# pyg-team/pytorch_geometric

Measured on AMD Instinct MI355X. Metric: edges/sec (fwd+bwd) 3-layer SAGE, ogbn-products shape, higher is better.
Workload: dtype f32

## Files before the change

include/pyg_amd.h:

```cpp
#ifndef PYG_AMD_H
#define PYG_AMD_H

#include <stddef.h>
#include <stdint.h>

#ifdef __cplusplus
extern "C" {
#endif

#define PYGAMD_API __attribute__((visibility("default")))

#define PYGAMD_ABI_VERSION 11

typedef enum {
  PYGAMD_OK = 0,
  PYGAMD_ERR_INVALID_ARG = 1,
  PYGAMD_ERR_UNSUPPORTED = 2,
  PYGAMD_ERR_WORKSPACE = 3,
  PYGAMD_ERR_HIP = 4
} pygamd_status;

typedef enum { PYGAMD_IDX_I32 = 0, PYGAMD_IDX_I64 = 1 } pygamd_idx_dtype;

typedef enum { PYGAMD_X_DENSE = 0, PYGAMD_X_COMPRESSED = 1 } pygamd_x_format;
// ... 429 lines not shown
                                                    const int64_t* frontier_time,
                                                    const int64_t* item_begin,
                                                    const int64_t* et_table, int n_et,
                                                    uint64_t timed_mask, int replace,
                                                    int strategy, void* lo_out, void* hi_out,
                                                    void* cnt_out, void* stream);
PYGAMD_API int pygamd_hetero_sample_neighbors_temporal(const void* row, const void* perm,
                                                       int idx_dtype, const void* frontier,
                                                       const void* lo, const void* hi,
                                                       const void* offsets,
                                                       const int64_t* item_begin,
                                                       const int64_t* et_table, int n_et,
                                                       uint64_t seed, int flags, void* src_out,
                                                       void* col_out, void* edge_out,
                                                       void* fpos_out, void* stream);

PYGAMD_API int pygamd_hetero_spmm(const void* rowptr, const void* col, int idx_dtype,
                                  const int64_t* row_begin, const float* const* x,
                                  float* const* out, const int64_t* et_table, int n_et, int64_t F,
                                  int32_t* err_flag, void* stream);
PYGAMD_API int pygamd_hetero_spmm_backward(const void* rowptr_t, const void* col_t,
                                           const void* rowptr, int idx_dtype,
                                           const int64_t* row_begin, const float* const* grad,
                                           const int64_t* et_table, int n_et,
                                           const int64_t* src_begin, float* const* grad_x,
                                           const int64_t* ld_grad_x, int n_nt, int64_t F,
                                           void* stream);

PYGAMD_API int pygamd_hgt_supported(int64_t H, int64_t D);
PYGAMD_API int pygamd_hgt_workspace_bytes(const int64_t* et_table, int n_et, int64_t H, int64_t D,
                                          size_t* bytes );
PYGAMD_API int pygamd_hgt_relation_forward(const float* const* k, const float* const* v,
                                           const int64_t* et_table, int n_et, const float* wk,
                                           const float* wv, int64_t T, int64_t H, int64_t D,
                                           float* kv, void* stream);
PYGAMD_API int pygamd_hgt_relation_backward(const float* const* k, const float* const* v,
                                            const int64_t* et_table, int n_et, const float* wk,
                                            const float* wv, int64_t T, int64_t H, int64_t D,
                                            const float* grad_kv, float* const* grad_k,
                                            float* const* grad_v, const int64_t* nt_table,
                                            int n_nt, float* grad_wk, float* grad_wv,
                                            void* workspace, size_t workspace_bytes,
                                            void* stream);

PYGAMD_API int pygamd_multi_reduce_csr(const void* rowptr, const void* perm, int idx_dtype,
                                       const float* x, int64_t ldx, int64_t n_rows, int64_t F,
                                       float* out_sum, float* out_sq, float* out_min,
                                       float* out_max, int64_t ldo, void* stream);

#define PYGAMD_GEMM_FP32 0
#define PYGAMD_GEMM_SPLIT_BF16 1
PYGAMD_API int pygamd_set_gemm_mode(int mode);
PYGAMD_API int pygamd_get_gemm_mode(void);
PYGAMD_API int pygamd_linear_nt_workspace_bytes(int64_t M, int64_t N_out, int64_t K_red,
                                                size_t* bytes );
PYGAMD_API int pygamd_linear_forward(const float* x, int64_t ldx, const float* w, int64_t ldw,
                                     const float* bias, int64_t M, int64_t K, int64_t N, int relu,
                                     int accumulate, float* out, int64_t ldo, void* workspace,
                                     size_t workspace_bytes, void* stream);
PYGAMD_API int pygamd_linear_dgrad(const float* g, int64_t ldg, const float* w_t, int64_t ldwt,
                                   const float* row_scale, int64_t n_scaled, int64_t M, int64_t N,
                                   int64_t K, int accumulate, const float* relu_mask,
                                   int64_t ld_mask, const uint32_t* relu_bits, int64_t ld_bits,
                                   float* out, int64_t ldo, void* stream);
PYGAMD_API int pygamd_linear_dgrad2(const float* g, int64_t ldg, const float* w_t, int64_t ldwt,
                                    const float* row_scale, int64_t n_scaled, int64_t M,
                                    int64_t N, int64_t K, int accumulate, const float* relu_mask,
                                    int64_t ld_mask, const uint32_t* relu_bits, int64_t ld_bits,
                                    float* out, int64_t ldo, float* out_scaled, int64_t ld_scaled,
                                    void* workspace, size_t workspace_bytes, void* stream);
PYGAMD_API int pygamd_linear_wgrad_workspace_bytes(int64_t M, int64_t N, int64_t K,
                                                   size_t* bytes );
PYGAMD_API int pygamd_linear_wgrad(const float* g, int64_t ldg, const float* x, int64_t ldx,
                                   int64_t M, int64_t N, int64_t K, int accumulate,
                                   int wgs_per_cu ,
                                   float* out, int64_t ldo, float* bias_grad, void* workspace,
                                   size_t workspace_bytes, void* stream);
PYGAMD_API int pygamd_linear_wgrad2(const float* g, int64_t ldg, const float* x, int64_t ldx,
                                    int64_t K1, const float* x2, int64_t ldx2, int64_t K2,
                                    int64_t M, int64_t N, int accumulate, int wgs_per_cu,
                                    float* out, int64_t ldo, float* bias_grad, void* workspace,
                                    size_t workspace_bytes, void* stream);

PYGAMD_API int pygamd_slots_max_fanout(void);
PYGAMD_API int pygamd_slots_max_hops(void);
PYGAMD_API int pygamd_slots_seed(const void* seeds, int idx_dtype, int64_t B,
                                 const int64_t* epoch_dev, int64_t* local_map, int64_t* node_g,
                                 void* stream);
PYGAMD_API int pygamd_slots_sample(const void* colptr, const void* row, int idx_dtype,
                                   const int64_t* node_g, int64_t frontier_base,
                                   int64_t n_frontier, int fanout, int64_t slot_base, int64_t B,
                                   uint64_t seed, int hop, const int64_t* epoch_dev,
                                   int64_t* local_map, int64_t* src_g, int32_t* row_end,
                                   float* inv_cnt, void* stream);
PYGAMD_API int pygamd_slots_resolve(const int64_t* src_g, int64_t slot_base, int64_t n_slots,
                                    int64_t B, const int64_t* epoch_dev,
                                    const int64_t* local_map, int32_t* src_id,
                                    int64_t* node_g, int32_t* const* counts ,
                                    int n_counts, void* stream);
PYGAMD_API int pygamd_slots_gather(const float* x, int64_t ldx, int64_t F, const int64_t* node_g,
                                   int64_t n_rows, float* out, int64_t ldo, void* stream);
PYGAMD_API int pygamd_slots_transpose(const int64_t* src_g, const int32_t* src_id, int hops,
                                      const int32_t* fanout ,
                                      const int64_t* bases , int n_csr,
                                      const int64_t* n_slots ,
                                      const int64_t* n_src_rows ,
// ... 65 lines not shown
```

pytorch_geometric_amd/_build.py:

```python
import os
import shutil
import subprocess
import sys
from concurrent.futures import ThreadPoolExecutor

PKG_DIR = os.path.dirname(os.path.abspath(__file__))
CSRC_DIR = os.path.join(PKG_DIR, 'csrc')
LIB_DIR = os.path.join(PKG_DIR, 'lib')
LIB_PATH = os.path.join(LIB_DIR, 'libpyg_amd.so')
LAB_LIB_PATH = os.path.join(LIB_DIR, 'libpyg_amd_lab.so')
BUILD_DIR = os.path.join(os.path.dirname(PKG_DIR), 'build', 'pyg_amd')
SOURCES = ['capi.hip', 'graph.hip', 'spmm.hip', 'scatter.hip', 'softmax.hip', 'segmm.hip',
           'sample.hip', 'minibatch.hip', 'train.hip', 'gemm.hip', 'sage_fused.hip',
           'hetero_conv.hip', 'gatv2.hip', 'transformer.hip', 'hgt.hip', 'gine.hip']
LAB_SOURCES = SOURCES + ['sage_fused_lab.hip']
LAB_FLAGS = {'gemm.hip': ['-DPYGAMD_LAB=1']}
ARCH = 'gfx950'
FLAGS = [f'--offload-arch={ARCH}', '-O3', '-std=c++17', '-fPIC', '-fvisibility=hidden',
         '-Wall', '-Wno-unused-function']
FLAGS += os.environ.get('PYGAMD_EXTRA_HIPCC_FLAGS', '').split()
EXTRA_FLAGS = {}


def find_hipcc():
    cand = shutil.which('hipcc') or '/opt/rocm/bin/hipcc'
    return cand if os.path.exists(cand) else None


STAMP_PATH = LIB_PATH + '.stamp'
LAB_STAMP_PATH = LAB_LIB_PATH + '.stamp'


BINDING_SRC = os.path.join(CSRC_DIR, 'torch_binding.cpp')
BINDING_PATH = os.path.join(LIB_DIR, 'libpyg_amd_torch.so')
BINDING_STAMP = BINDING_PATH + '.stamp'


def source_hash():
    import hashlib
    h = hashlib.sha1()
    paths = sorted(os.path.join(CSRC_DIR, f) for f in os.listdir(CSRC_DIR)
                   if f != os.path.basename(BINDING_SRC))
    paths.append(os.path.join(os.path.dirname(PKG_DIR), 'include', 'pyg_amd.h'))
    paths.append(os.path.join(os.path.dirname(PKG_DIR), 'include', 'pyg_amd_lab.h'))
    for p in paths:
        if os.path.isfile(p):
            h.update(os.path.basename(p).encode())
            with open(p, 'rb') as f:
                h.update(f.read())
    h.update(' '.join(FLAGS).encode())
    h.update(repr(sorted(EXTRA_FLAGS.items())).encode())
    return h.hexdigest()


def is_stale():
    if not (os.path.exists(LIB_PATH) and os.path.exists(STAMP_PATH)):
        return True
    with open(STAMP_PATH) as f:
        return f.read().strip() != source_hash()


def lab_is_stale():
    if not (os.path.exists(LAB_LIB_PATH) and os.path.exists(LAB_STAMP_PATH)):
        return True
    with open(LAB_STAMP_PATH) as f:
        return f.read().strip() != source_hash()
# ... 110 lines not shown
```

pytorch_geometric_amd/_lib.py:

```python
import ctypes
import os
from ctypes import (POINTER, Structure, c_char_p, c_double, c_float, c_int, c_int32, c_int64,
                    c_size_t, c_uint64, c_void_p)

from . import _build

ABI_VERSION = 11
X_DENSE, X_COMPRESSED = 0, 1
AGG_GIVEN = 2
IDX_I32, IDX_I64 = 0, 1
SUM, MEAN, MIN, MAX, MUL, ANY = 0, 1, 2, 3, 4, 5
REDUCE_IDS = {'sum': SUM, 'add': SUM, 'mean': MEAN, 'min': MIN, 'amin': MIN, 'max': MAX,
              'amax': MAX, 'mul': MUL, 'any': ANY}


class PygAmdError(RuntimeError):
    pass


class SpmmArgs(Structure):
    _fields_ = [
        ('rowptr', c_void_p), ('col', c_void_p), ('eid', c_void_p), ('w', c_void_p),
        ('src_scale', c_void_p), ('x', c_void_p), ('out', c_void_p), ('arg_out', c_void_p),
        ('n_rows', c_int64), ('n_src', c_int64), ('F', c_int64), ('ldx', c_int64),
# ... 41 lines not shown
    'pygamd_ptr2index': (c_int, [_P, c_int, c_int64, c_int64, _P, _P]),
    'pygamd_index_minmax': (c_int, [_P, c_int, c_int64, _P, _P]),
    'pygamd_permute_index': (c_int, [_P, c_int, _P, c_int64, _P, _P]),
    'pygamd_cast_index': (c_int, [_P, c_int64, c_int, _P, _P]),
    'pygamd_index_guard': (c_int, [_P, c_int, c_int64, c_int64, _P, c_int, _P, _P]),
    'pygamd_cumsum_workspace_bytes': (c_int, [c_int, c_int64, POINTER(c_size_t)]),
    'pygamd_cumsum': (c_int, [_P, c_int, c_int64, _P, _P, c_size_t, _P]),
    'pygamd_hub_plan_workspace_bytes': (c_int, [c_int, c_int64, POINTER(c_size_t)]),
    'pygamd_hub_plan': (c_int, [_P, c_int, c_int64, c_int64, c_int64, _P, _P, c_int64,
                                POINTER(c_int64), POINTER(c_int64), _P, c_size_t, _P]),
    'pygamd_rows_compress': (c_int, [_P, c_int64, c_int64, c_int64, _P, c_int64, _P]),
    'pygamd_rows_pack': (c_int, [_P, c_int64, c_int64, c_int64, _P, _P, c_int64, c_int64, _P,
                                 c_int64, c_int64, _P, _P, _P]),
    'pygamd_spmm_csr_workspace_bytes': (c_int, [POINTER(SpmmArgs), POINTER(c_size_t)]),
    'pygamd_spmm_csr': (c_int, [POINTER(SpmmArgs), _P, c_size_t, _P]),
    'pygamd_spmm_csr_tie_count': (c_int, [_P, _P, c_int, _P, c_int64, _P, c_int64, c_int64,
                                          c_int64, c_int, _P, _P]),
    'pygamd_spmm_csr_minmax_backward': (c_int, [_P, _P, c_int, _P, c_int64, _P, _P, _P, c_int64,
                                                c_int64, c_int64, _P, c_int64, _P]),
    'pygamd_spmm_csr_minmax_backward_dst': (c_int, [_P, _P, c_int, _P, c_int64, _P, c_int64, _P,
                                                    c_int64, c_int64, c_int64, c_int64, c_int, _P,
                                                    c_int64, _P]),
    'pygamd_multi_reduce_csr': (c_int, [_P, _P, c_int, _P, c_int64, c_int64, c_int64, _P, _P, _P,
                                        _P, c_int64, _P]),
    'pygamd_minmax_backward_src_workspace_bytes': (c_size_t, [c_int64, c_int64, c_int64]),
    'pygamd_spmm_csr_minmax_backward_src': (c_int, [_P, _P, _P, _P, _P, c_int, _P, _P, c_int64, _P,
                                                    c_int64, _P, c_int64, c_int64, c_int64,
                                                    c_int64, c_int64, c_int, _P, c_size_t, _P,
                                                    c_int64, _P]),
    'pygamd_spmm_csr_minmax_backward_arg': (c_int, [_P, _P, c_int, _P, _P, c_int64, _P, c_int64, _P,
                                                    c_int64, c_int64, c_int64, c_int64, c_int, _P,
                                                    c_int64, _P]),
    'pygamd_sddmm_csr': (c_int, [_P, _P, _P, c_int, _P, c_int64, _P, c_int64, c_int64, c_int64,
                                 c_int32, c_int32, _P, _P]),
    'pygamd_sddmm_spmm_csr': (c_int, [_P, _P, _P, c_int, _P, c_int64, _P, c_int64, c_int64,
                                      c_int64, c_int32, c_int32, _P, _P, _P, c_int64, _P]),
    'pygamd_colsum': (c_int, [_P, c_int64, c_int64, c_int64, _P, _P]),
    'pygamd_bias_act': (c_int, [_P, c_int64, _P, c_int64, c_int64, c_int, _P, c_int64, _P]),
    'pygamd_relu_backward_colsum': (c_int, [_P, c_int64, _P, c_int64, c_int64, c_int64, _P,
                                            c_int64, _P, _P]),
    'pygamd_sage_layer_forward_supported': (c_int, [c_int64, c_int64, c_int]),
    'pygamd_sage_layer_forward': (c_int, [POINTER(SpmmArgs), _P, c_int64, _P, c_int64, _P, c_int64,
                                          c_int, c_int, _P, c_int64, _P, c_int64, _P, c_size_t,
                                          _P]),
    'pygamd_sage_layer_fused': (c_int, [POINTER(SpmmArgs), POINTER(SageFusedArgs), _P, c_size_t,
                                        _P]),
    'pygamd_sage_layer_fused_workspace_bytes': (c_int, [POINTER(SpmmArgs), POINTER(SageFusedArgs),
                                                        POINTER(c_size_t)]),
    'pygamd_linear_nt_workspace_bytes': (c_int, [c_int64, c_int64, c_int64, POINTER(c_size_t)]),
    'pygamd_linear_forward': (c_int, [_P, c_int64, _P, c_int64, _P, c_int64, c_int64, c_int64,
                                      c_int, c_int, _P, c_int64, _P, c_size_t, _P]),
    'pygamd_set_gemm_mode': (c_int, [c_int]),
    'pygamd_get_gemm_mode': (c_int, []),
    'pygamd_linear_dgrad': (c_int, [_P, c_int64, _P, c_int64, _P, c_int64, c_int64, c_int64,
                                    c_int64, c_int, _P, c_int64, _P, c_int64, _P, c_int64, _P]),
    'pygamd_linear_dgrad2': (c_int, [_P, c_int64, _P, c_int64, _P, c_int64, c_int64, c_int64,
                                     c_int64, c_int, _P, c_int64, _P, c_int64, _P, c_int64, _P,
                                     c_int64, _P, c_size_t, _P]),
    'pygamd_linear_wgrad_workspace_bytes': (c_int, [c_int64, c_int64, c_int64,
                                                    POINTER(c_size_t)]),
    'pygamd_linear_wgrad': (c_int, [_P, c_int64, _P, c_int64, c_int64, c_int64, c_int64, c_int,
                                    c_int, _P, c_int64, _P, _P, c_size_t, _P]),
    'pygamd_linear_wgrad2': (c_int, [_P, c_int64, _P, c_int64, c_int64, _P, c_int64, c_int64,
                                     c_int64, c_int64, c_int, c_int, _P, c_int64, _P, _P,
                                     c_size_t, _P]),
    'pygamd_segment_matmul_tile_rows': (c_int, []),
    'pygamd_segment_matmul_workspace_bytes': (c_int, [c_int64, c_int64, c_int64,
                                                      POINTER(c_size_t)]),
    'pygamd_segment_matmul': (c_int, [_P, c_int64, _P, _P, c_int64, c_int64, c_int64, c_int64,
                                      _P, c_int64, c_int64, c_int64, c_int64, _P, c_int64, _P,
                                      c_size_t, _P]),
    'pygamd_segment_matmul_wgrad': (c_int, [_P, c_int64, _P, c_int64, _P, _P, c_int64, c_int64,
                                            c_int64, c_int64, c_int64, _P, _P]),
    'pygamd_sample_max_fanout': (c_int, []),
    'pygamd_sample_neighbors': (c_int, [_P, _P, c_int, _P, c_int64, _P, c_int64, c_uint64, c_int,
                                        _P, _P, _P, _P, _P]),
    'pygamd_sample_neighbors_weighted': (c_int, [_P, _P, c_int, _P, _P, c_int64, _P, c_int64,
                                                 c_uint64, c_int, _P, _P, _P, _P, _P]),
    'pygamd_sample_temporal_window': (c_int, [_P, _P, c_int, _P, c_int, _P, _P, c_int64, c_int64,
                                              c_int, c_int, _P, _P, _P, _P, _P]),
    'pygamd_sample_neighbors_temporal': (c_int, [_P, c_int, _P, c_int64, _P, _P, _P, c_int64,
                                                 c_uint64, c_int, _P, _P, _P, _P, _P]),
    'pygamd_slots_max_fanout': (c_int, []),
    'pygamd_slots_max_hops': (c_int, []),
    'pygamd_slots_seed': (c_int, [_P, c_int, c_int64, _P, _P, _P, _P]),
    'pygamd_slots_sample': (c_int, [_P, _P, c_int, _P, c_int64, c_int64, c_int, c_int64, c_int64,
                                    c_uint64, c_int, _P, _P, _P, _P, _P, _P]),
    'pygamd_slots_resolve': (c_int, [_P, c_int64, c_int64, c_int64, _P, _P, _P, _P, _P, c_int,
                                     _P]),
    'pygamd_slots_gather': (c_int, [_P, c_int64, c_int64, _P, c_int64, _P, c_int64, _P]),
    'pygamd_slots_transpose': (c_int, [_P, _P, c_int, _P, _P, c_int, _P, _P, _P, _P, _P, _P, _P]),
    'pygamd_cross_entropy_step_workspace_bytes': (c_int, [c_int64, _P]),
    'pygamd_cross_entropy_step': (c_int, [_P, c_int64, _P, c_int64, c_int64, c_int64, _P, _P, _P,
                                          c_int64, _P, _P, c_size_t, _P, _P, _P]),
    'pygamd_adam_step': (c_int, [_P, _P, _P, _P, c_int64, _P, c_int64, c_double, c_double,
                                 c_double, c_double, c_double, c_double, _P, c_int, _P, _P, _P,
                                 _P, _P]),
    'pygamd_edge_key': (c_int, [_P, _P, c_int, c_int64, c_int64, c_int, _P, _P]),
    'pygamd_run_flags': (c_int, [_P, c_int64, _P, _P]),
    'pygamd_edge_unkey': (c_int, [_P, _P, _P, c_int64, c_int64, c_int, c_int, _P, _P, _P, _P]),
    'pygamd_sample_counts': (c_int, [_P, c_int, _P, c_int64, c_int64, c_int, _P, _P, _P]),
    'pygamd_relabel': (c_int, [c_int, _P, c_int, c_int64, _P, _P, _P, c_int64, _P, _P, _P]),
    'pygamd_sample_negatives': (c_int, [c_int64, c_int64, c_uint64, _P, _P, _P, _P, c_int64,
                                        c_int64, c_int, _P, _P]),
    'pygamd_unique_inverse': (c_int, [_P, _P, c_int, c_int64, _P, _P, c_size_t, _P, _P, _P, _P]),
    'pygamd_hetero_sample_counts': (c_int, [_P, c_int, _P, _P, _P, c_int, c_int, _P, _P]),
# ... 53 lines not shown
                                                 c_int64, c_float, _P, _P, _P]),
    'pygamd_gatv2_supported': (c_int, [c_int64, c_int64]),
    'pygamd_gatv2_workspace_bytes': (c_int, [c_int64, c_int64, c_int64, POINTER(c_size_t)]),
    'pygamd_gatv2_forward': (c_int, [_G, _P, _P, _P, c_int64, c_int64, c_int64, c_float, _P, _P, _P,
                                     c_size_t, _P]),
    'pygamd_gatv2_backward_dst': (c_int, [_G, _P, _P, _P, _P, _P, _P, _P, c_int64, c_int64, c_int64,
                                          c_float, _P, _P, _P, _P, c_size_t, _P]),
    'pygamd_gatv2_backward_src': (c_int, [_G, _P, _P, _P, _P, _P, _P, _P, c_int64, c_int64, c_int64,
                                          c_float, _P, _P, c_size_t, _P]),
    'pygamd_transformer_supported': (c_int, [c_int64, c_int64]),
    'pygamd_transformer_workspace_bytes': (c_int, [c_int64, c_int64, c_int64,
                                                   POINTER(c_size_t)]),
    'pygamd_transformer_forward': (c_int, [_G, _P, _P, _P, c_int64, c_int64, c_int64, c_int64,
                                           c_float, _P, _P, _P, c_size_t, _P]),
    'pygamd_transformer_backward_dst': (c_int, [_G, _P, _P, c_int64, _P, _P, _P, _P, c_int64,
                                                c_int64, c_int64, c_float, _P, _P, _P, c_size_t,
                                                _P]),
    'pygamd_transformer_backward_src': (c_int, [_G, _P, _P, _P, _P, _P, c_int64, c_int64, c_int64,
                                                c_float, _P, _P, c_int64, _P, c_size_t, _P]),
    'pygamd_transformer_edge_supported': (c_int, [c_int64, c_int64, c_int64]),
    'pygamd_transformer_edge_workspace_bytes': (c_int, [c_int64, c_int64, c_int64, c_int64,
                                                        POINTER(c_size_t)]),
    'pygamd_transformer_edge_forward': (c_int, [_G, _P, _P, _P, c_int64, _P, _P, c_int64, c_int64,
                                                c_int64, c_int64, c_float, _P, _P, _P, _P, c_size_t,
                                                _P]),
    'pygamd_transformer_edge_backward_dst': (c_int, [_G, _P, _P, c_int64, _P, _P, _P, _P, _P, _P,
                                                     _P, _P, c_int64, c_int64, c_int64, c_int64,
                                                     c_float, _P, _P, _P, _P, _P, c_size_t, _P]),
    'pygamd_gine_supported': (c_int, [c_int64, c_int64]),
    'pygamd_gine_workspace_bytes': (c_int, [c_int64, c_int64, c_int64, POINTER(c_size_t)]),
    'pygamd_gine_forward': (c_int, [_G, _P, _P, c_int64, _P, c_int64, _P, _P, _P, _P, c_int64,
                                    c_int64, c_int64, _P, _P, c_size_t, _P]),
    'pygamd_gine_backward': (c_int, [_G, _P, _P, c_int64, _P, _P, _P, _P, c_int64, c_int64, c_int64,
                                     _P, _P, _P, _P, _P, c_size_t, _P]),
}

LAB_SIGNATURES = {
    'pygamd_lab_sage_layer_fused': (c_int, [POINTER(SpmmArgs), POINTER(SageFusedArgs), c_int,
                                            c_int, _P, c_size_t, _P]),
    'pygamd_lab_set_wgrad_variant': (c_int, [c_int]),
    'pygamd_lab_copy': (c_int, [_P, _P, c_int64, c_int, c_int, _P]),
}

_lib = None
_lab = None
_use_lab = False


def lib_path():
    return _build.LIB_PATH


GEMM_MODES = {'fp32': 0, 'split': 1}


def _open(path, signatures):
    lib = ctypes.CDLL(path)
    for name, (restype, argtypes) in signatures:
        fn = getattr(lib, name)
        fn.restype = restype
        fn.argtypes = argtypes
    if lib.pygamd_abi_version() != ABI_VERSION:
        raise PygAmdError(f'ABI mismatch: {path} reports {lib.pygamd_abi_version()}')
    return lib


def _default_mode():
    mode = os.environ.get('PYGAMD_GEMM_MODE', 'split')
    if mode not in GEMM_MODES:
        raise PygAmdError(f"PYGAMD_GEMM_MODE must be one of {sorted(GEMM_MODES)}, got '{mode}'")
    return GEMM_MODES[mode]


def load():
    global _lib
    if _use_lab:
        return load_lab()
    if _lib is not None:
        return _lib
    path = _build.LIB_PATH
    if _build.is_stale():
        if _build.find_hipcc() is not None and os.environ.get('PYG_AMD_NO_BUILD') != '1':
            _build.build_library(verbose=False)
        elif not os.path.exists(path):
            raise PygAmdError(
                f"{path} is missing and hipcc is unavailable: run "
                f"`python -c 'import __graft_entry__ as g; g.build()'` on a machine with ROCm. "
                f"There is no CPU fallback for the pytorch_geometric_amd kernels.")
    lib = _open(path, list(SIGNATURES.items()))
    lib.pygamd_set_gemm_mode(_default_mode())
    _lib = lib
    return lib


def load_lab():
    global _lab
    if _lab is not None:
        return _lab
    path = _build.LAB_LIB_PATH
    if _build.lab_is_stale():
        if _build.find_hipcc() is not None and os.environ.get('PYG_AMD_NO_BUILD') != '1':
            _build.build_lab_library(verbose=False)
        elif not os.path.exists(path):
            raise PygAmdError(f"{path} is missing and hipcc is unavailable (the laboratory "
                              f"build: `python -m pytorch_geometric_amd._build`)")
    lab = _open(path, list(SIGNATURES.items()) + list(LAB_SIGNATURES.items()))
    lab.pygamd_set_gemm_mode(_lib.pygamd_get_gemm_mode() if _lib is not None else _default_mode())
    _lab = lab
    return lab


def use_lab(flag: bool) -> None:
    global _use_lab
    _use_lab = bool(flag)
    if _use_lab:
        load_lab()


def lab_active() -> bool:
    return _use_lab


def loaded():
    if _lib is None and _lab is None:
        load()
    return [l for l in (_lib, _lab) if l is not None]


def check(rc, what=''):
    if rc != 0:
        lib = load()
        msg = lib.pygamd_status_string(rc).decode()
        extra = f' (hipError {lib.pygamd_last_hip_error()})' if rc == 4 else ''
        raise PygAmdError(f'{what or "pygamd call"} failed: {msg}{extra}')
```

pytorch_geometric_amd/_native.py:

```python
import collections
import ctypes
import os
import threading
from typing import Optional, Tuple

import torch
from torch import Tensor

from . import _compiled, _lib
from ._lib import REDUCE_IDS, Csr, PygAmdError, SpmmArgs, check

HUB_THRESHOLD = 1024
HUB_CHUNK = int(os.environ.get('PYGAMD_HUB_CHUNK', '256'))


def _require_device(*tensors):
    for t in tensors:
        if t is not None and not t.is_cuda:
            raise PygAmdError(
                'pytorch_geometric_amd kernels need HIP device tensors (got a '
                f'{t.device} tensor); there is no CPU fallback on this path')


def _idx_dtype(t: Tensor) -> int:
# ... 1623 lines not shown
                                     'compressed_out': compressed_out is not None}}, ev0, ev1))
    return out


def cross_entropy_rows(logits: Tensor, target: Tensor, index: Optional[Tensor] = None):
    _require_device(logits, target, index)
    x = _f32_rows(logits, 'logits')
    N, C = x.shape
    if target.dtype != torch.int64 or target.dim() != 1 or target.numel() != N \
            or not target.is_contiguous():
        raise ValueError(f"'target' must hold one contiguous int64 label per row of 'logits' "
                         f"({N}), got {target.dtype} {tuple(target.shape)}")
    if index is not None and (index.dtype != torch.int64 or index.dim() != 1
                              or not index.is_contiguous()):
        raise ValueError("'index' must be a contiguous 1-D int64 tensor")
    B = N if index is None else index.numel()
    if B == 0 or C == 0:
        raise ValueError('cross_entropy_rows needs at least one row and one class')
    lib = _lib.load()
    grad = torch.empty(B, C, dtype=torch.float32, device=x.device)
    loss = torch.empty((), dtype=torch.float32, device=x.device)
    nbytes = ctypes.c_size_t(0)
    check(lib.pygamd_cross_entropy_step_workspace_bytes(B, ctypes.byref(nbytes)))
    ws = torch.empty(nbytes.value, dtype=torch.uint8, device=x.device)
    ring, slot, err = _index_flag(x.device, True)
    check(lib.pygamd_cross_entropy_step(_p(x), _ld(x), _p(index), N, B, C, _p(target), _p(index),
                                        _p(grad), C, _p(loss), _p(ws), nbytes.value, _p(err),
                                        None, _stream(x)), 'cross_entropy_rows')
    _index_flag_done(ring, slot, err, "cross_entropy: a target outside [0, C) (or an 'index' "
                     "entry outside the rows of the logits)", C, target)
    return loss, grad


def set_gemm_mode(mode: str) -> str:
    lib = _lib.load()
    if mode not in _lib.GEMM_MODES:
        raise ValueError(f"mode must be one of {sorted(_lib.GEMM_MODES)}, got '{mode}'")
    prev = get_gemm_mode()
    for each in _lib.loaded():
        check(each.pygamd_set_gemm_mode(_lib.GEMM_MODES[mode]), 'set_gemm_mode')
    return prev


def lab_set_wgrad_variant(variant: int) -> None:
    check(_lib.load_lab().pygamd_lab_set_wgrad_variant(int(variant)), 'lab_set_wgrad_variant')
    _lib.use_lab(int(variant) != 0)


def get_gemm_mode() -> str:
    code = _lib.load().pygamd_get_gemm_mode()
    return next(k for k, v in _lib.GEMM_MODES.items() if v == code)


def linear_dgrad(g: Tensor, w_t: Tensor, row_scale: Optional[Tensor] = None, n_scaled: int = 0,
                 out: Optional[Tensor] = None, accumulate: bool = False,
                 relu_mask: Optional[Tensor] = None, relu_bits: Optional[Tensor] = None,
                 out_scaled: Optional[Tensor] = None) -> Tensor:
    _require_device(g, w_t, row_scale, out, relu_mask, relu_bits, out_scaled)
    if relu_mask is not None and relu_bits is not None:
        raise ValueError("pass at most one of 'relu_mask' / 'relu_bits'")
    C = _compiled.ops()
    if C is not None and _plain(g, w_t, relu_mask, out, out_scaled) \
            and g.size(1) == w_t.size(1):
        M, K = g.size(0), w_t.size(0)
        ok = ((out is None or (out.shape == (M, K) and (K <= 1 or out.stride(1) == 1)))
              and (relu_mask is None or tuple(relu_mask.shape) == (M, K))
              and (out_scaled is None or (row_scale is not None and not accumulate
                                          and out_scaled.shape == (M, K)
                                          and (K <= 1 or out_scaled.stride(1) == 1))))
        if ok:
            _check_bits(relu_bits, M, K)
            if out is None:
                out = torch.empty(M, K, dtype=torch.float32, device=g.device)
            with _timed({'kind': 'gemm', 'op': 'dgrad', 'M': M, 'N': K, 'K': g.size(1)}, g):
                C.linear_dgrad(g, w_t, row_scale, n_scaled, out, accumulate, relu_mask,
                               relu_bits, out_scaled)
            return out
    lib = _lib.load()
    g2, w2 = _f32_rows(g, 'grad'), _f32_rows(w_t, 'weight_t')
    M, N = g2.shape
    K = w2.size(0)
    if w2.size(1) != N:
        raise ValueError(f"'grad' has {N} columns but 'weight_t' expects {w2.size(1)}")
    if out is None:
        out = torch.empty(M, K, dtype=torch.float32, device=g.device)
    if row_scale is not None:
        row_scale = row_scale.contiguous()
    if out_scaled is not None:
        if row_scale is None or accumulate:
            raise ValueError("'out_scaled' needs 'row_scale' and no 'accumulate'")
        if out_scaled.shape != (M, K) or out_scaled.dtype != torch.float32 \
                or (K > 1 and out_scaled.stride(1) != 1):
            raise ValueError("'out_scaled' must be a float32 [M, K] tensor with unit inner stride")
    m2 = None
    _check_bits(relu_bits, M, K)
    if relu_mask is not None:
        m2 = _f32_rows(relu_mask, 'relu_mask')
        if tuple(m2.shape) != (M, K):
            raise ValueError(f"'relu_mask' must be [{M}, {K}], got {tuple(m2.shape)}")
    ws, ws_bytes = _nt_workspace(lib, M, K, N, g.device)
    with _timed({'kind': 'gemm', 'op': 'dgrad', 'M': M, 'N': K, 'K': N}, g):
        check(lib.pygamd_linear_dgrad2(_p(g2), _ld(g2), _p(w2), _ld(w2), _p(row_scale),
                                       n_scaled if row_scale is not None else 0, M, N, K,
                                       int(accumulate), _p(m2), _ld(m2) if m2 is not None else 0,
                                       _p(relu_bits),
                                       relu_bits.size(1) if relu_bits is not None else 0,
# ... 795 lines not shown
```

pytorch_geometric_amd/csrc/gemm.hip:

```cpp
#include "split_bf16.h"
#include "../../include/pyg_amd_lab.h"

namespace pygamd {

typedef float f32x16 __attribute__((ext_vector_type(16)));
typedef float f32x4 __attribute__((ext_vector_type(4)));

struct SplitFrag {
  bf16x8 p[3];
};

__device__ __forceinline__ SplitFrag split_frag(const f32x4& v0, const f32x4& v1) {
  u32x4 w[3];
#pragma unroll
  for (int q = 0; q < 4; ++q) {
    const float x0 = q < 2 ? v0[2 * q] : v1[2 * q - 4];
    const float x1 = q < 2 ? v0[2 * q + 1] : v1[2 * q - 3];
    uint32_t t[3];
    split_pair(x0, x1, t);
    w[0][q] = t[0];
    w[1][q] = t[1];
    w[2][q] = t[2];
  }
  SplitFrag f;
#pragma unroll
  for (int t = 0; t < 3; ++t) f.p[t] = __builtin_bit_cast(bf16x8, w[t]);
  return f;
}

__device__ __forceinline__ void split_term(int t, const SplitFrag& a, const SplitFrag& b,
                                           f32x16& acc) {
  acc = __builtin_amdgcn_mfma_f32_32x32x16_bf16(a.p[kSplitTa[t]], b.p[kSplitTb[t]], acc, 0, 0, 0);
}

constexpr int kGK = 32;
constexpr int kGLD = kGK + 4;

struct GemmNT {
  const float* __restrict__ a;
  const float* __restrict__ b;
  const float* __restrict__ bias;
  const float* __restrict__ row_scale;
  const float* __restrict__ mask;
  const uint32_t* __restrict__ mask_bits;
  int64_t ldmb;
  float* __restrict__ c;
  float* __restrict__ c2;
  int64_t ldc2;
  int64_t M, lda, ldb, ldc, ldm;
  int N, K;
  int relu;
  int n_scaled;
  int accumulate;
  int tiles_m, tiles_n;
  int split;
  int ksplits, k_per_split;
  float* __restrict__ partial;
};

__device__ __forceinline__ void nt_tile_of_block(const GemmNT& p, int& tm, int& tn) {
  const int64_t b = blockIdx.x;
  const int64_t per_xcd = gridDim.x >> 3;
  const int64_t q = (b & 7) * per_xcd + (b >> 3);
  tm = static_cast<int>(q / p.tiles_n);
  tn = static_cast<int>(q - static_cast<int64_t>(tm) * p.tiles_n);
}

template <int WM, int WN, int TM, int TN, bool VEC, bool SPLIT>
__global__ void __launch_bounds__(kBlock, 2) gemm_nt_kernel(GemmNT p) {
  static_assert(WM * WN == 4, "four waves per workgroup");
  constexpr int BM = WM * TM * 32, BN = WN * TN * 32;
  constexpr int A_LD4 = BM * (kGK / 4) / kBlock;
  constexpr int B_LD4 = (BN * (kGK / 4) + kBlock - 1) / kBlock;
  extern __shared__ __align__(16) float smem[];
  float* As = smem;
  float* Bs = smem + 2 * BM * kGLD;
  int tile_m, tile_n;
  nt_tile_of_block(p, tile_m, tile_n);
  if (tile_m >= p.tiles_m) return;
  const int64_t m0 = static_cast<int64_t>(tile_m) * BM;
  const int n0 = tile_n * BN;
  const int wave = threadIdx.x >> 6, lane = threadIdx.x & 63;
  const int wm = wave / WN, wn = wave % WN;
  const int li = lane & 31, lh = lane >> 5;
  const int kb = p.ksplits > 1 ? static_cast<int>(blockIdx.y) * p.k_per_split : 0;
  const int ke = p.ksplits > 1 ? (kb + p.k_per_split < p.K ? kb + p.k_per_split : p.K) : p.K;

  const int kq = threadIdx.x & 7;
  const int r0 = threadIdx.x >> 3;
  const float* pa[A_LD4];
  const float* pb[B_LD4];
  bool okb[B_LD4];
#pragma unroll
  for (int q = 0; q < A_LD4; ++q) {
    int64_t row = m0 + r0 + 32 * q;
    row = row < p.M ? row : p.M - 1;
    pa[q] = p.a + row * p.lda;
  }
#pragma unroll
  for (int q = 0; q < B_LD4; ++q) {
    int row = n0 + r0 + 32 * q;
    okb[q] = row < p.N && (BN % 32 == 0 || r0 + 32 * q < BN);
    row = row < p.N ? row : p.N - 1;
    pb[q] = p.b + static_cast<int64_t>(row) * p.ldb;
  }
  f32x4 ra[A_LD4], rb[B_LD4];
  auto load_chunk = [&](int k0) {
    const int k = k0 + 4 * kq;
    if (VEC) {
      const int kc = k < ke ? k : 0;
#pragma unroll
// ... 1076 lines not shown
  return PYGAMD_OK;
}

static int g_gemm_mode = 0;
#ifdef PYGAMD_LAB
static int g_wgrad_variant = 0;
#else
constexpr int g_wgrad_variant = 0;
#endif

constexpr int kFillTiles = 128;
struct NtShape {
  int tile;
  int ksplits;
  int k_per_split;
};
static NtShape nt_shape(int64_t M, int N, int K, bool allow_splitk) {
  NtShape s;
  s.tile = N > 96 ? 0 : N > 64 ? 1 : N > 32 ? 2 : 3;
  s.ksplits = 1;
  s.k_per_split = K;
  const int bn[5] = {128, 96, 64, 32, 64};
  int64_t tiles = ceil_div(M, 128) * ceil_div(N, bn[s.tile]);
  if (tiles >= kFillTiles) return s;
  if (N > 32) {
    s.tile = 4;
    tiles = ceil_div(M, 64) * ceil_div(N, 64);
  }
  if (allow_splitk && tiles < kFillTiles && K >= 128) {
    int want = static_cast<int>(ceil_div(2 * kFillTiles, tiles));
    const int most = K / 64;
    want = want < most ? want : most;
    want = want < 32 ? want : 32;
    if (want > 1) {
      s.k_per_split = static_cast<int>(round_up(ceil_div(K, want), kGK));
      s.ksplits = static_cast<int>(ceil_div(K, s.k_per_split));
    }
  }
  return s;
}

static int run_nt(GemmNT p, void* workspace, size_t workspace_bytes, hipStream_t st) {
  if (p.M == 0 || p.N == 0) return PYGAMD_OK;
  p.split = g_gemm_mode == PYGAMD_GEMM_SPLIT_BF16 ? 1 : 0;
  const bool vec = (p.K % 4 == 0) && (p.lda % 4 == 0) && (p.ldb % 4 == 0) && aligned16p(p.a) &&
                   aligned16p(p.b);
  NtShape sh = nt_shape(p.M, p.N, p.K, workspace != nullptr);
  if (sh.ksplits > 1 &&
      workspace_bytes < static_cast<size_t>(sh.ksplits) * p.M * p.N * sizeof(float))
    sh = nt_shape(p.M, p.N, p.K, false);
  p.ksplits = sh.ksplits;
  p.k_per_split = sh.k_per_split;
  p.partial = sh.ksplits > 1 ? static_cast<float*>(workspace) : nullptr;
  switch (sh.tile) {
    case 0: return launch_nt<2, 2, 2, 2>(p, vec, st);
    case 1: return launch_nt<4, 1, 1, 3>(p, vec, st);
    case 2: return launch_nt<4, 1, 1, 2>(p, vec, st);
    case 3: return launch_nt<4, 1, 1, 1>(p, vec, st);
    default: return launch_nt<2, 2, 1, 1>(p, vec, st);
  }
}

}

using namespace pygamd;

extern "C" {

int pygamd_set_gemm_mode(int mode) {
  if (mode != PYGAMD_GEMM_FP32 && mode != PYGAMD_GEMM_SPLIT_BF16) return PYGAMD_ERR_INVALID_ARG;
  g_gemm_mode = mode;
  return PYGAMD_OK;
}

int pygamd_get_gemm_mode(void) { return g_gemm_mode; }

#ifdef PYGAMD_LAB
int pygamd_lab_set_wgrad_variant(int variant) {
  if (variant < 0 || variant > 127 || ((variant & 1) && variant != 1))
    return PYGAMD_ERR_INVALID_ARG;
  g_wgrad_variant = variant;
  return PYGAMD_OK;
}
#endif

int pygamd_linear_forward(const float* x, int64_t ldx, const float* w, int64_t ldw,
                          const float* bias, int64_t M, int64_t K, int64_t N, int relu,
                          int accumulate, float* out, int64_t ldo, void* workspace,
                          size_t workspace_bytes, void* stream) {
  if (M < 0 || K < 0 || N < 0 || K > INT32_MAX || N > INT32_MAX || ldx < K || ldw < K ||
      ldo < N)
    return PYGAMD_ERR_INVALID_ARG;
  if (M == 0 || N == 0) return PYGAMD_OK;
  if (!out || (K > 0 && (!x || !w))) return PYGAMD_ERR_INVALID_ARG;
  GemmNT p = {};
  p.a = x; p.b = w; p.bias = bias; p.row_scale = nullptr; p.mask = nullptr; p.c = out;
  p.M = M; p.lda = ldx; p.ldb = ldw; p.ldc = ldo; p.ldm = 0;
  p.N = static_cast<int>(N); p.K = static_cast<int>(K);
  p.relu = relu ? 1 : 0; p.n_scaled = 0; p.accumulate = accumulate ? 1 : 0;
  return run_nt(p, workspace, workspace_bytes, as_stream(stream));
}

int pygamd_linear_dgrad2(const float* g, int64_t ldg, const float* w_t, int64_t ldwt,
                         const float* row_scale, int64_t n_scaled, int64_t M, int64_t N,
                         int64_t K, int accumulate, const float* relu_mask, int64_t ld_mask,
                         const uint32_t* relu_bits, int64_t ld_bits, float* out, int64_t ldo,
// ... 186 lines not shown
```

Baseline: 4.503 billion.

## Add persistent streaming NT GEMM kernel with LDS-resident split-bf16 weights

```diff
diff --git a/include/pyg_amd.h b/include/pyg_amd.h
--- a/include/pyg_amd.h
+++ b/include/pyg_amd.h
@@ -505,6 +505,12 @@
 #define PYGAMD_GEMM_SPLIT_BF16 1
 PYGAMD_API int pygamd_set_gemm_mode(int mode);
 PYGAMD_API int pygamd_get_gemm_mode(void);
+#define PYGAMD_STREAM_OFF 0
+#define PYGAMD_STREAM_AUTO 1
+#define PYGAMD_STREAM_FORCE 2
+PYGAMD_API int pygamd_set_stream_mode(int mode);
+PYGAMD_API int pygamd_get_stream_mode(void);
+PYGAMD_API int64_t pygamd_stream_launch_count(void);
 PYGAMD_API int pygamd_linear_nt_workspace_bytes(int64_t M, int64_t N_out, int64_t K_red,
                                                 size_t* bytes );
 PYGAMD_API int pygamd_linear_forward(const float* x, int64_t ldx, const float* w, int64_t ldw,
diff --git a/pytorch_geometric_amd/_build.py b/pytorch_geometric_amd/_build.py
--- a/pytorch_geometric_amd/_build.py
+++ b/pytorch_geometric_amd/_build.py
@@ -11,7 +11,7 @@
 LAB_LIB_PATH = os.path.join(LIB_DIR, 'libpyg_amd_lab.so')
 BUILD_DIR = os.path.join(os.path.dirname(PKG_DIR), 'build', 'pyg_amd')
 SOURCES = ['capi.hip', 'graph.hip', 'spmm.hip', 'scatter.hip', 'softmax.hip', 'segmm.hip',
-           'sample.hip', 'minibatch.hip', 'train.hip', 'gemm.hip', 'sage_fused.hip',
+           'sample.hip', 'minibatch.hip', 'train.hip', 'gemm.hip', 'stream_nt.hip', 'sage_fused.hip',
            'hetero_conv.hip', 'gatv2.hip', 'transformer.hip', 'hgt.hip', 'gine.hip']
 LAB_SOURCES = SOURCES + ['sage_fused_lab.hip']
 LAB_FLAGS = {'gemm.hip': ['-DPYGAMD_LAB=1']}
diff --git a/pytorch_geometric_amd/_lib.py b/pytorch_geometric_amd/_lib.py
--- a/pytorch_geometric_amd/_lib.py
+++ b/pytorch_geometric_amd/_lib.py
@@ -117,6 +117,9 @@
                                       c_int, c_int, _P, c_int64, _P, c_size_t, _P]),
     'pygamd_set_gemm_mode': (c_int, [c_int]),
     'pygamd_get_gemm_mode': (c_int, []),
+    'pygamd_set_stream_mode': (c_int, [c_int]),
+    'pygamd_get_stream_mode': (c_int, []),
+    'pygamd_stream_launch_count': (c_int64, []),
     'pygamd_linear_dgrad': (c_int, [_P, c_int64, _P, c_int64, _P, c_int64, c_int64, c_int64,
                                     c_int64, c_int, _P, c_int64, _P, c_int64, _P, c_int64, _P]),
     'pygamd_linear_dgrad2': (c_int, [_P, c_int64, _P, c_int64, _P, c_int64, c_int64, c_int64,
@@ -276,6 +279,7 @@
 
 
 GEMM_MODES = {'fp32': 0, 'split': 1}
+STREAM_MODES = {'off': 0, 'auto': 1, 'force': 2}
 
 
 def _open(path, signatures):
@@ -294,6 +298,14 @@
     if mode not in GEMM_MODES:
         raise PygAmdError(f"PYGAMD_GEMM_MODE must be one of {sorted(GEMM_MODES)}, got '{mode}'")
     return GEMM_MODES[mode]
+
+
+def _default_stream_mode():
+    mode = os.environ.get('PYGAMD_STREAM_MODE', 'auto')
+    if mode not in STREAM_MODES:
+        raise PygAmdError(f"PYGAMD_STREAM_MODE must be one of {sorted(STREAM_MODES)}, got "
+                          f"'{mode}'")
+    return STREAM_MODES[mode]
 
 
 def load():
@@ -313,6 +325,7 @@
                 f"There is no CPU fallback for the pytorch_geometric_amd kernels.")
     lib = _open(path, list(SIGNATURES.items()))
     lib.pygamd_set_gemm_mode(_default_mode())
+    lib.pygamd_set_stream_mode(_default_stream_mode())
     _lib = lib
     return lib
 
@@ -330,6 +343,8 @@
                               f"build: `python -m pytorch_geometric_amd._build`)")
     lab = _open(path, list(SIGNATURES.items()) + list(LAB_SIGNATURES.items()))
     lab.pygamd_set_gemm_mode(_lib.pygamd_get_gemm_mode() if _lib is not None else _default_mode())
+    lab.pygamd_set_stream_mode(_lib.pygamd_get_stream_mode() if _lib is not None
+                               else _default_stream_mode())
     _lab = lab
     return lab
 
diff --git a/pytorch_geometric_amd/_native.py b/pytorch_geometric_amd/_native.py
--- a/pytorch_geometric_amd/_native.py
+++ b/pytorch_geometric_amd/_native.py
@@ -1699,6 +1699,25 @@
     return next(k for k, v in _lib.GEMM_MODES.items() if v == code)
 
 
+def set_stream_mode(mode: str) -> str:
+    _lib.load()
+    if mode not in _lib.STREAM_MODES:
+        raise ValueError(f"mode must be one of {sorted(_lib.STREAM_MODES)}, got '{mode}'")
+    prev = get_stream_mode()
+    for each in _lib.loaded():
+        check(each.pygamd_set_stream_mode(_lib.STREAM_MODES[mode]), 'set_stream_mode')
+    return prev
+
+
+def get_stream_mode() -> str:
+    code = _lib.load().pygamd_get_stream_mode()
+    return next(k for k, v in _lib.STREAM_MODES.items() if v == code)
+
+
+def stream_launch_count() -> int:
+    return int(_lib.load().pygamd_stream_launch_count())
+
+
 def linear_dgrad(g: Tensor, w_t: Tensor, row_scale: Optional[Tensor] = None, n_scaled: int = 0,
                  out: Optional[Tensor] = None, accumulate: bool = False,
                  relu_mask: Optional[Tensor] = None, relu_bits: Optional[Tensor] = None,
diff --git a/pytorch_geometric_amd/csrc/gemm.hip b/pytorch_geometric_amd/csrc/gemm.hip
--- a/pytorch_geometric_amd/csrc/gemm.hip
+++ b/pytorch_geometric_amd/csrc/gemm.hip
@@ -1,62 +1,10 @@
-#include "split_bf16.h"
+#include "gemm_nt.h"
 #include "../../include/pyg_amd_lab.h"
 
 namespace pygamd {
-
-typedef float f32x16 __attribute__((ext_vector_type(16)));
-typedef float f32x4 __attribute__((ext_vector_type(4)));
-
-struct SplitFrag {
-  bf16x8 p[3];
-};
-
-__device__ __forceinline__ SplitFrag split_frag(const f32x4& v0, const f32x4& v1) {
-  u32x4 w[3];
-#pragma unroll
-  for (int q = 0; q < 4; ++q) {
-    const float x0 = q < 2 ? v0[2 * q] : v1[2 * q - 4];
-    const float x1 = q < 2 ? v0[2 * q + 1] : v1[2 * q - 3];
-    uint32_t t[3];
-    split_pair(x0, x1, t);
-    w[0][q] = t[0];
-    w[1][q] = t[1];
-    w[2][q] = t[2];
-  }
-  SplitFrag f;
-#pragma unroll
-  for (int t = 0; t < 3; ++t) f.p[t] = __builtin_bit_cast(bf16x8, w[t]);
-  return f;
-}
-
-__device__ __forceinline__ void split_term(int t, const SplitFrag& a, const SplitFrag& b,
-                                           f32x16& acc) {
-  acc = __builtin_amdgcn_mfma_f32_32x32x16_bf16(a.p[kSplitTa[t]], b.p[kSplitTb[t]], acc, 0, 0, 0);
-}
 
 constexpr int kGK = 32;
 constexpr int kGLD = kGK + 4;
-
-struct GemmNT {
-  const float* __restrict__ a;
-  const float* __restrict__ b;
-  const float* __restrict__ bias;
-  const float* __restrict__ row_scale;
-  const float* __restrict__ mask;
-  const uint32_t* __restrict__ mask_bits;
-  int64_t ldmb;
-  float* __restrict__ c;
-  float* __restrict__ c2;
-  int64_t ldc2;
-  int64_t M, lda, ldb, ldc, ldm;
-  int N, K;
-  int relu;
-  int n_scaled;
-  int accumulate;
-  int tiles_m, tiles_n;
-  int split;
-  int ksplits, k_per_split;
-  float* __restrict__ partial;
-};
 
 __device__ __forceinline__ void nt_tile_of_block(const GemmNT& p, int& tm, int& tn) {
   const int64_t b = blockIdx.x;
@@ -1239,6 +1187,7 @@
   p.ksplits = sh.ksplits;
   p.k_per_split = sh.k_per_split;
   p.partial = sh.ksplits > 1 ? static_cast<float*>(workspace) : nullptr;
+  if (stream_nt_takes(p, vec)) return stream_nt_launch(p, st);
   switch (sh.tile) {
     case 0: return launch_nt<2, 2, 2, 2>(p, vec, st);
     case 1: return launch_nt<4, 1, 1, 3>(p, vec, st);
diff --git a/pytorch_geometric_amd/csrc/gemm_nt.h b/pytorch_geometric_amd/csrc/gemm_nt.h
--- /dev/null
+++ b/pytorch_geometric_amd/csrc/gemm_nt.h
@@ -0,0 +1,61 @@
+#pragma once
+#include "split_bf16.h"
+
+namespace pygamd {
+
+typedef float f32x16 __attribute__((ext_vector_type(16)));
+typedef float f32x4 __attribute__((ext_vector_type(4)));
+
+struct SplitFrag {
+  bf16x8 p[3];
+};
+
+__device__ __forceinline__ SplitFrag split_frag(const f32x4& v0, const f32x4& v1) {
+  u32x4 w[3];
+#pragma unroll
+  for (int q = 0; q < 4; ++q) {
+    const float x0 = q < 2 ? v0[2 * q] : v1[2 * q - 4];
+    const float x1 = q < 2 ? v0[2 * q + 1] : v1[2 * q - 3];
+    uint32_t t[3];
+    split_pair(x0, x1, t);
+    w[0][q] = t[0];
+    w[1][q] = t[1];
+    w[2][q] = t[2];
+  }
+  SplitFrag f;
+#pragma unroll
+  for (int t = 0; t < 3; ++t) f.p[t] = __builtin_bit_cast(bf16x8, w[t]);
+  return f;
+}
+
+__device__ __forceinline__ void split_term(int t, const SplitFrag& a, const SplitFrag& b,
+                                           f32x16& acc) {
+  acc = __builtin_amdgcn_mfma_f32_32x32x16_bf16(a.p[kSplitTa[t]], b.p[kSplitTb[t]], acc, 0, 0, 0);
+}
+
+struct GemmNT {
+  const float* __restrict__ a;
+  const float* __restrict__ b;
+  const float* __restrict__ bias;
+  const float* __restrict__ row_scale;
+  const float* __restrict__ mask;
+  const uint32_t* __restrict__ mask_bits;
+  int64_t ldmb;
+  float* __restrict__ c;
+  float* __restrict__ c2;
+  int64_t ldc2;
+  int64_t M, lda, ldb, ldc, ldm;
+  int N, K;
+  int relu;
+  int n_scaled;
+  int accumulate;
+  int tiles_m, tiles_n;
+  int split;
+  int ksplits, k_per_split;
+  float* __restrict__ partial;
+};
+
+bool stream_nt_takes(const GemmNT& p, bool vec);
+int stream_nt_launch(const GemmNT& p, hipStream_t st);
+
+}
diff --git a/pytorch_geometric_amd/csrc/stream_nt.hip b/pytorch_geometric_amd/csrc/stream_nt.hip
--- /dev/null
+++ b/pytorch_geometric_amd/csrc/stream_nt.hip
@@ -0,0 +1,261 @@
+#include <atomic>
+
+#include "gemm_nt.h"
+
+namespace pygamd {
+
+constexpr int kSnThreads = 512;
+constexpr int kSnWaves = kSnThreads / kWave;
+constexpr size_t kSnLdsMax = 160 * 1024;
+
+__host__ __device__ constexpr int sn_row_quads(int K) { return K / 8 + 1; }
+constexpr size_t sn_lds_bytes(int N, int K) {
+  return static_cast<size_t>(3) * N * sn_row_quads(K) * 16;
+}
+
+template <int NC, int TN, int WN, bool SLICED>
+__global__ void __launch_bounds__(kSnThreads) stream_nt_kernel(GemmNT p) {
+  constexpr int K = 32 * NC, N = 32 * TN * WN;
+  constexpr int WM = kSnWaves / WN, BM = 32 * WM;
+  constexpr int RING = NC <= 4 ? NC : 4;
+  static_assert(NC % RING == 0, "a ring slot holds the same chunks of every tile");
+  static_assert(sn_lds_bytes(N, K) <= kSnLdsMax, "the weight planes stay in LDS");
+  constexpr int QS = sn_row_quads(K);
+  extern __shared__ __align__(16) u32x4 sn_planes[];
+
+  for (int i = threadIdx.x; i < N * (K / 8); i += kSnThreads) {
+    const int n = i / (K / 8), q = i - n * (K / 8);
+    const float* wp = p.b + static_cast<int64_t>(n) * p.ldb + 8 * q;
+    const SplitFrag f =
+        split_frag(*reinterpret_cast<const f32x4*>(wp), *reinterpret_cast<const f32x4*>(wp + 4));
+#pragma unroll
+    for (int t = 0; t < 3; ++t)
+      sn_planes[(t * N + n) * QS + q] = __builtin_bit_cast(u32x4, f.p[t]);
+  }
+  __syncthreads();
+
+  const int wave = __builtin_amdgcn_readfirstlane(static_cast<int>(threadIdx.x >> 6));
+  const int lane = threadIdx.x & 63;
+  const int wm = wave / WN, wn = wave % WN;
+  const int li = lane & 31, lh = lane >> 5;
+
+  const int64_t tiles = (p.M + BM - 1) / BM;
+  const int64_t base = tiles / gridDim.x, rem = tiles % gridDim.x;
+  const int64_t bid = blockIdx.x;
+  const int64_t t0 = bid * base + (bid < rem ? bid : rem);
+  const int64_t nt = base + (bid < rem ? 1 : 0);
+  if (nt == 0) return;
+
+  auto row_ptr = [&](int64_t t) {
+    int64_t row = t * BM + wm * 32 + li;
+    row = row < p.M ? row : p.M - 1;
+    return p.a + row * p.lda + 16 * lh;
+  };
+  f32x4 raw[RING][4];
+  auto load_chunk = [&](f32x4 (&r)[4], const float* rp, int c) {
+#pragma unroll
+    for (int v = 0; v < 4; ++v) r[v] = *reinterpret_cast<const f32x4*>(rp + 32 * c + 4 * v);
+  };
+  const u32x4* const bq = sn_planes + (wn * TN * 32 + li) * QS + 2 * lh;
+  auto read_b = [&](SplitFrag (&sb)[TN], int c, int hf) {
+#pragma unroll
+    for (int j = 0; j < TN; ++j)
+#pragma unroll
+      for (int t = 0; t < 3; ++t)
+        sb[j].p[t] = __builtin_bit_cast(bf16x8, bq[(t * N + j * 32) * QS + 4 * c + hf]);
+  };
+
+  float bv[TN];
+#pragma unroll
+  for (int j = 0; j < TN; ++j) bv[j] = p.bias ? p.bias[(wn * TN + j) * 32 + li] : 0.f;
+  const bool want_scale = p.n_scaled > 0 || p.c2;
+
+  const float* cur = row_ptr(t0);
+#pragma unroll
+  for (int c = 0; c < RING; ++c) load_chunk(raw[c], cur, c);
+
+  for (int64_t t = t0; t < t0 + nt; ++t) {
+    const float* const nxt = row_ptr(t + 1);
+    const int64_t rb0 = t * BM + wm * 32;
+    const int64_t rbase = rb0 + 4 * lh;
+    const bool full = rb0 + 32 <= p.M;
+    const bool use_sc = full && want_scale, use_bits = full && p.mask_bits != nullptr;
+    const float* const scp = use_sc ? p.row_scale + rbase : p.a + 4 * lh;
+    const uint32_t* const wdp =
+        use_bits ? p.mask_bits + ((rb0 >> 5) * p.ldmb + wn * TN) * 32 + li
+                 : reinterpret_cast<const uint32_t*>(p.a) + li;
+    const int wstep = use_bits ? 32 : 0;
+    f32x4 sc[4];
+    uint32_t word[TN];
+#pragma unroll
+    for (int g4 = 0; g4 < 4; ++g4)
+#pragma unroll
+      for (int e = 0; e < 4; ++e) sc[g4][e] = scp[8 * g4 + e];
+#pragma unroll
+    for (int j = 0; j < TN; ++j) word[j] = wdp[j * wstep];
+    __builtin_amdgcn_sched_barrier(0);
+    f32x16 acc[TN], tot[SLICED ? TN : 1];
+#pragma unroll
+    for (int j = 0; j < TN; ++j)
+#pragma unroll
+      for (int e = 0; e < 16; ++e) acc[j][e] = 0.f;
+    if constexpr (SLICED) {
+#pragma unroll
+      for (int j = 0; j < TN; ++j)
+#pragma unroll
+        for (int e = 0; e < 16; ++e) tot[j][e] = 0.f;
+    }
+#pragma unroll
+    for (int c = 0; c < NC; ++c) {
+      f32x4(&r)[4] = raw[c % RING];
+      const SplitFrag sa0 = split_frag(r[0], r[1]);
+      const SplitFrag sa1 = split_frag(r[2], r[3]);
+      __builtin_amdgcn_sched_barrier(0);
+      if (c + RING < NC) load_chunk(r, cur, c + RING);
+      else load_chunk(r, nxt, c + RING - NC);
+      __builtin_amdgcn_sched_barrier(0);
+      SplitFrag sb[TN];
+      read_b(sb, c, 0);
+#pragma unroll
+      for (int s = 0; s < kSplitTerms; ++s)
+#pragma unroll
+        for (int j = 0; j < TN; ++j) split_term(s, sa0, sb[j], acc[j]);
+      read_b(sb, c, 1);
+#pragma unroll
+      for (int s = 0; s < kSplitTerms; ++s)
+#pragma unroll
+        for (int j = 0; j < TN; ++j) split_term(s, sa1, sb[j], acc[j]);
+      if constexpr (SLICED) {
+        if (c == NC - 1 || (32 * (c + 1)) % p.k_per_split == 0) {
+#pragma unroll
+          for (int j = 0; j < TN; ++j)
+#pragma unroll
+            for (int e = 0; e < 16; ++e) {
+              tot[j][e] += acc[j][e];
+              acc[j][e] = c == NC - 1 ? tot[j][e] : 0.f;
+            }
+        }
+      }
+    }
+    cur = nxt;
+
+    if (rb0 >= p.M) continue;
+    if (full) {
+#pragma unroll
+      for (int j = 0; j < TN; ++j) {
+        const int col = (wn * TN + j) * 32 + li;
+        const bool scaled = col < p.n_scaled;
+        float* cp = p.c + rbase * p.ldc + col;
+        float* cp2 = p.c2 ? p.c2 + rbase * p.ldc2 + col : nullptr;
+        auto emit = [&](auto keep) {
+#pragma unroll
+          for (int e = 0; e < 16; ++e) {
+            float v = acc[j][e] + bv[j];
+            if (p.n_scaled > 0) v = scaled ? v * sc[e >> 2][e & 3] : v;
+            if (p.relu) v = (v > 0.f || v != v) ? v : 0.f;
+            v = keep(e) ? v : 0.f;
+            cp[((e & 3) + 8 * (e >> 2)) * p.ldc] = v;
+            if (cp2) cp2[((e & 3) + 8 * (e >> 2)) * p.ldc2] = v * sc[e >> 2][e & 3];
+          }
+        };
+        if (p.mask_bits) {
+          uint32_t bw[16];
+#pragma unroll
+          for (int e = 0; e < 16; ++e)
+            bw[e] = __shfl(word[j], (e & 3) + 8 * (e >> 2) + 4 * lh, kWave);
+          emit([&](int e) { return ((bw[e] >> li) & 1u) != 0; });
+        } else {
+          emit([](int) { return true; });
+        }
+      }
+      continue;
+    }
+#pragma unroll
+    for (int j = 0; j < TN; ++j) {
+      const int col = (wn * TN + j) * 32 + li;
+      const bool scaled = col < p.n_scaled;
+#pragma unroll
+      for (int e = 0; e < 16; ++e) {
+        const int64_t row = rbase + (e & 3) + 8 * (e >> 2);
+        if (row < p.M) {
+          float v = acc[j][e] + bv[j];
+          if (scaled) v *= p.row_scale[row];
+          if (p.relu) v = (v > 0.f || v != v) ? v : 0.f;
+          if (p.mask_bits)
+            v = ((p.mask_bits[((row >> 5) * p.ldmb + (col >> 5)) * 32 + (row & 31)] >> (col & 31)) &
+                 1u)
+                    ? v
+                    : 0.f;
+          p.c[row * p.ldc + col] = v;
+          if (p.c2) p.c2[row * p.ldc2 + col] = v * p.row_scale[row];
+        }
+      }
+    }
+  }
+}
+
+static int g_stream_mode = PYGAMD_STREAM_AUTO;
+static std::atomic<int64_t> g_stream_launches{0};
+
+static int sn_shape(int N, int K) {
+  if (K == 256 && N == 96) return 1;
+  if (K == 96 && N == 256) return 2;
+  return 0;
+}
+
+constexpr int64_t kSnMinRows = 32768;
+
+bool stream_nt_takes(const GemmNT& p, bool vec) {
+  if (g_stream_mode == PYGAMD_STREAM_OFF || !p.split || !vec || p.accumulate || p.mask) return false;
+  const int shape = sn_shape(p.N, p.K);
+  if (shape == 0 || (shape == 2 && p.ksplits > 1)) return false;
+  return g_stream_mode == PYGAMD_STREAM_FORCE || p.M >= kSnMinRows;
+}
+
+template <int NC, int TN, int WN, bool SLICED = false>
+static int sn_launch(const GemmNT& p, hipStream_t st) {
+  constexpr int BM = 32 * (kSnWaves / WN);
+  constexpr size_t lds = sn_lds_bytes(32 * TN * WN, 32 * NC);
+  int dev = 0, cus = 0;
+  PYGAMD_HIP_CHECK(hipGetDevice(&dev));
+  PYGAMD_HIP_CHECK(hipDeviceGetAttribute(&cus, hipDeviceAttributeMultiprocessorCount, dev));
+  const int64_t tiles = ceil_div(p.M, BM);
+  const int64_t grid = tiles < cus ? tiles : cus;
+  void (*k)(GemmNT) = stream_nt_kernel<NC, TN, WN, SLICED>;
+  PYGAMD_HIP_CHECK(hipFuncSetAttribute(reinterpret_cast<const void*>(k),
+                                       hipFuncAttributeMaxDynamicSharedMemorySize,
+                                       static_cast<int>(lds)));
+  hipLaunchKernelGGL(k, dim3(static_cast<unsigned>(grid)), dim3(kSnThreads), lds, st, p);
+  PYGAMD_LAUNCH_CHECK();
+  g_stream_launches.fetch_add(1, std::memory_order_relaxed);
+  return PYGAMD_OK;
+}
+
+int stream_nt_launch(const GemmNT& p, hipStream_t st) {
+  switch (sn_shape(p.N, p.K)) {
+    case 1: return p.ksplits > 1 ? sn_launch<8, 3, 1, true>(p, st) : sn_launch<8, 3, 1>(p, st);
+    case 2: return p.ksplits > 1 ? PYGAMD_ERR_INVALID_ARG : sn_launch<3, 4, 2>(p, st);
+    default: return PYGAMD_ERR_INVALID_ARG;
+  }
+}
+
+}
+
+using namespace pygamd;
+
+extern "C" {
+
+int pygamd_set_stream_mode(int mode) {
+  if (mode != PYGAMD_STREAM_OFF && mode != PYGAMD_STREAM_AUTO && mode != PYGAMD_STREAM_FORCE)
+    return PYGAMD_ERR_INVALID_ARG;
+  g_stream_mode = mode;
+  return PYGAMD_OK;
+}
+
+int pygamd_get_stream_mode(void) { return g_stream_mode; }
+
+int64_t pygamd_stream_launch_count(void) {
+  return g_stream_launches.load(std::memory_order_relaxed);
+}
+
+}
```

Measured after the change: 4.548 billion, median of 6. No clear change (+1.0%).
